# AOADMM-DataFusionFramework/Matlab-Code

Hardware: AMD Instinct MI355X
Metric: AO-ADMM outer iters/sec (+ mode-1 MTTKRP GFLOP/s), 2000^3 rank-20 CP (higher is better)
Workload: dtype f32

## Files before the change

### matlab-code_amd/csrc/contract.h

```cpp
#pragma once
#include "common.h"

namespace aoadmm {

struct DenseTensor {
  int prec = AOADMM_PREC_F64;
  int nd = 0;
  int64_t dims[8] = {0};
  int64_t pad0 = 0;
  DevBuf data;
  int64_t elems_padded() const {
    int64_t n = pad0;
    for (int i = 1; i < nd; ++i) n *= dims[i];
    return n;
  }
  size_t elem_size() const { return prec == AOADMM_PREC_F32 ? 4 : 8; }
};

struct ContractPlan {
  int64_t nbatch, batch_stride, M, ld, C;
  int R;
  int tprec = AOADMM_PREC_F64;
  int nchunk;
  bool lead = false;
  bool on_copy = false;
  int64_t trows() const { return nbatch * M; }
  size_t t_bytes() const { return (size_t)nchunk * trows() * R * (tprec == AOADMM_PREC_F32 ? 4 : 8); }
  size_t frag_bytes(int prec) const;
  double algorithmic_bytes(int prec) const {
    return (double)nbatch * M * C * (prec == AOADMM_PREC_F32 ? 4.0 : 8.0) + (double)t_bytes();
  }
  double flops() const { return 2.0 * nbatch * M * C * R; }
};

ContractPlan make_plan(int64_t nbatch, int64_t batch_stride, int64_t M, int64_t ld, int64_t C, int R,
                       int prec);

ContractPlan make_lead_plan(int64_t M, int64_t ld, int64_t C, int R);

void launch_contract(const void* X, int prec, const ContractPlan& pl, const double* F, int64_t ldF,
                     void* frag_ws, void* T, hipStream_t s, hipEvent_t ev0 = nullptr,
                     hipEvent_t ev1 = nullptr);

size_t reduce_factor_scratch_bytes(int64_t rows, int R);
struct SysBuild;
bool launch_reduce_inner(const void* T, int tprec, int nchunk, int64_t trows, int64_t A, int64_t Apad,
                         int64_t B, int R, const double* Fa, int64_t ldFa, double scale,
                         double* out, int64_t ldOut, double* ft_scratch, hipStream_t s,
                         const double* FaT = nullptr,
                         int rowmajor_out = 0,
                         const SysBuild* sys = nullptr);
size_t reduce_outer_scratch_bytes(int64_t A, int64_t B, int R);
bool launch_reduce_outer(const void* T, int tprec, int nchunk, int64_t trows, int64_t A, int64_t Apad,
                         int64_t B, int R, const double* Fb, int64_t ldFb, double scale,
                         double* out, int64_t ldOut, double* scratch, double* ft_scratch, hipStream_t s,
                         const double* FbT = nullptr, int rowmajor_out = 0, const SysBuild* sys = nullptr);
void launch_t_to_colmajor(const void* T, int tprec, int nchunk, int64_t trows, int64_t A, int R, double scale,
                          double* out, int64_t ldOut, hipStream_t s);

constexpr int64_t kSmallMttkrpElems = (int64_t)1 << 19;
struct SmallMttkrp {
  const void* X;
  int64_t sn, sa, sb;
  int Na, Nb, R;
  const double *Fa, *Fb;
  int64_t lda, ldb;
  double scale;
  double* out;
  int64_t ldOut;
};
bool small_mttkrp_ok(int64_t elems, int nd, const int64_t* dims, int R);
// ... 4 lines not shown
```

### matlab-code_amd/csrc/contract.hip

```cpp
#include "contract.h"
#include "device_utils.h"
#include "small_dev.h"

#include <algorithm>
#include <cstdlib>

namespace aoadmm {

typedef float f32x4 __attribute__((ext_vector_type(4)));
typedef double f64x2 __attribute__((ext_vector_type(2)));
typedef double f64x4 __attribute__((ext_vector_type(4)));

static constexpr int kTileRows = 128;
static constexpr int kGroup = 8;

struct KArgs {
  const void* X;
  const void* frag;
  void* T;
  int64_t tiles_per_batch, ntiles, batch_stride, M, ld, C, Cg, trows;
  int groups_per_chunk, R;
  int flush_every;
};

typedef float f32x2 __attribute__((ext_vector_type(2)));

__global__ void pack_frag16_f32(const double* __restrict__ F, int64_t ldF, int64_t C, int R, int NT, int EX,
                                int64_t Cg, float* __restrict__ frag) {
  const int64_t idx = (int64_t)blockIdx.x * blockDim.x + threadIdx.x;
  const int64_t nmain = (int64_t)NT * Cg * 128;
  if (idx < nmain) {
    const int kk = idx & 1;
    const int lane = (idx >> 1) & 63;
    const int64_t g = (idx >> 7) % Cg;
    const int nt = (int)((idx >> 7) / Cg);
    const int64_t c = 8 * g + 4 * kk + (lane >> 4);
    const int r = 16 * nt + (lane & 15);
// ... 6 lines not shown
    const int r = 16 * NT + e;
    frag[idx] = (c < C && r < R) ? (float)F[c + ldF * r] : 0.f;
  }
}

__device__ __forceinline__ float quarter_sum4(float a, float b, float c, float d) {
  const auto ab = __builtin_amdgcn_permlane16_swap(__float_as_uint(a), __float_as_uint(b), false, false);
  const auto cd = __builtin_amdgcn_permlane16_swap(__float_as_uint(c), __float_as_uint(d), false, false);
  const float s_ab = __uint_as_float(ab[0]) + __uint_as_float(ab[1]);
  const float s_cd = __uint_as_float(cd[0]) + __uint_as_float(cd[1]);
  const auto x = __builtin_amdgcn_permlane32_swap(__float_as_uint(s_ab), __float_as_uint(s_cd), false, false);
  return __uint_as_float(x[0]) + __uint_as_float(x[1]);
}

constexpr int kFlushEvery = 3;
template <int NT, bool EX, bool L2 = false>
__global__ __launch_bounds__(256, NT <= 2 ? 2 : 1) void contract16_f32(KArgs a) {
  static_assert(!L2 || NT == 1, "two-level accumulation exists for one 16-column tile (R <= 20)");
  const int lane = threadIdx.x & 63;
  const int64_t wt = (int64_t)blockIdx.x * 4 + (threadIdx.x >> 6);
  if (wt >= a.ntiles) return;
  const int chunk = blockIdx.y;
  const int64_t b = wt / a.tiles_per_batch;
  const int64_t m0 = (wt - b * a.tiles_per_batch) * kTileRows;
  const int r16 = lane & 15, q = lane >> 4;
  int64_t row0 = m0 + 4 * r16, row1 = m0 + 64 + 4 * r16;
  if (row0 >= a.M) row0 = m0;
  if (row1 >= a.M) row1 = m0;
  const int64_t g0 = (int64_t)chunk * a.groups_per_chunk;
  int64_t g1 = g0 + a.groups_per_chunk;
  if (g1 > a.Cg) g1 = a.Cg;
  const int64_t gfull = (a.C / kGroup < g1) ? a.C / kGroup : g1;
  const float* X = reinterpret_cast<const float*>(a.X) + b * a.batch_stride;
// ... 189 lines not shown
#pragma unroll
      for (int h = 0; h < 2; ++h)
#pragma unroll
        for (int v = 0; v < 4; ++v)
#pragma unroll
          for (int e = 0; e < 4; ++e)
            if (e < ne) tl[(64 * h + 4 * r16 + v) * a.R + 16 * NT + e] = accE[h][v][e >> 1][e & 1];
    }
  }
  {
    const int64_t rows_here = (a.M - m0 < kTileRows) ? a.M - m0 : kTileRows;
    const int n16 = (int)(rows_here * a.R / 4);
    f32x4* dst = reinterpret_cast<f32x4*>(reinterpret_cast<float*>(a.T) + ((int64_t)chunk * a.trows + b * a.M + m0) * a.R);
    const f32x4* src = reinterpret_cast<const f32x4*>(tl);
    for (int c = lane; c < n16; c += 64) __builtin_nontemporal_store(src[c], dst + c);
  }
}

static constexpr int kLeadRows = 128;
static constexpr int kLeadKC = 64;
static constexpr int kLeadStride = 68;

struct LArgs {
  const float* X;
  const float* frag;
  float* T;
  int64_t M, ld, C, Cg;
  int chunks_per_slice;
  int R;
};
// ... 392 lines not shown
  if (nt16 == 1) AO_SET(contract_lead16_f32<1>)
  else if (nt16 == 2) AO_SET(contract_lead16_f32<2>)
  else if (nt16 == 3) AO_SET(contract_lead16_f32<3>)
  else if (nt16 == 4) AO_SET(contract_lead16_f32<4>)
#undef AO_SET
  if (ev0) AO_HIP(hipEventRecord(ev0, s));
  if (nt16 == 1) contract_lead16_f32<1><<<grid, 256, sh, s>>>(a);
  else if (nt16 == 2) contract_lead16_f32<2><<<grid, 256, sh, s>>>(a);
  else if (nt16 == 3) contract_lead16_f32<3><<<grid, 256, sh, s>>>(a);
  else if (nt16 == 4) contract_lead16_f32<4><<<grid, 256, sh, s>>>(a);
  else throw Error(AOADMM_ERR_UNSUPPORTED, "rank > 64 not supported");
  if (ev1) AO_HIP(hipEventRecord(ev1, s));
  AO_KERNEL_CHECK();
}

void launch_contract(const void* X, int prec, const ContractPlan& pl, const double* F, int64_t ldF,
                     void* frag_ws, void* T, hipStream_t s, hipEvent_t ev0, hipEvent_t ev1) {
  AO_REQUIRE(pl.tprec == prec, "contraction plan and tensor precision disagree");
  AO_REQUIRE(pl.R >= 1 && pl.R <= kMaxRank, "rank %d outside [1,%d]", pl.R, kMaxRank);
  if (pl.lead) {
    AO_REQUIRE(prec == AOADMM_PREC_F32, "leading-mode contraction exists for fp32 tensors only");
    launch_contract_lead(X, pl, F, ldF, frag_ws, T, s, ev0, ev1);
    return;
  }
  const int64_t Cg = cdiv(pl.C, kGroup);
  KArgs a;
  a.X = X; a.frag = frag_ws; a.T = T;
  a.tiles_per_batch = cdiv(pl.M, tile_rows(prec));
  a.ntiles = pl.nbatch * a.tiles_per_batch;
  a.batch_stride = pl.batch_stride; a.M = pl.M; a.ld = pl.ld; a.C = pl.C; a.Cg = Cg;
  a.trows = pl.trows();
  a.groups_per_chunk = (int)cdiv(Cg, pl.nchunk);
  a.R = pl.R;
  AO_REQUIRE(a.ntiles > 0 && pl.C > 0, "empty contraction");
  dim3 grid((unsigned)cdiv(a.ntiles, 4), (unsigned)pl.nchunk);
  AO_REQUIRE(cdiv(a.ntiles, 4) < (int64_t)2147483647, "tensor too large for one launch");
  if (prec == AOADMM_PREC_F32) {
    AO_REQUIRE(pl.ld % 4 == 0 && pl.M % 4 == 0 && pl.batch_stride % 4 == 0, "f32 layout must be padded to 4");
    const int rem = pl.R % 16;
    const bool ex = pl.R > 16 && rem >= 1 && rem <= 4;
    const int nt16 = ex ? pl.R / 16 : (pl.R + 15) / 16;
    const int64_t total = (int64_t)nt16 * Cg * 128 + (ex ? Cg * 32 : 0);
    pack_frag16_f32<<<(unsigned)cdiv(total, 256), 256, 0, s>>>(F, ldF, pl.C, pl.R, nt16, ex ? 1 : 0, Cg, (float*)frag_ws);
    AO_KERNEL_CHECK();
    size_t tsh = (size_t)4 * kTileRows * pl.R * sizeof(float);
    a.flush_every = kFlushEvery;
    if (nt16 == 1) tsh = (size_t)4 * 16384;
#define AO_GO(K) { if (tsh > 65536) ensure_dynamic_lds(reinterpret_cast<const void*>(K), (int)tsh); if (ev0) AO_HIP(hipEventRecord(ev0, s)); K<<<grid, 256, tsh, s>>>(a); }
    if (nt16 == 1 && !ex) AO_GO((contract16_f32<1, false, true>))
    else if (nt16 == 1) AO_GO((contract16_f32<1, true, true>))
    else if (nt16 == 2 && !ex) AO_GO((contract16_f32<2, false>))
    else if (nt16 == 2) AO_GO((contract16_f32<2, true>))
    else if (nt16 == 3 && !ex) AO_GO((contract16_f32<3, false>))
    else if (nt16 == 3) AO_GO((contract16_f32<3, true>))
    else if (nt16 == 4) AO_GO((contract16_f32<4, false>))
    else throw Error(AOADMM_ERR_UNSUPPORTED, "rank > 64 not supported");
#undef AO_GO
  } else {
    AO_REQUIRE(pl.ld % 2 == 0 && pl.M % 2 == 0 && pl.batch_stride % 2 == 0, "f64 layout must be padded to 2");
    const int rem = pl.R % 16;
    const bool ex = pl.R > 16 && rem >= 1 && rem <= 4;
    const int nt16 = ex ? pl.R / 16 : (pl.R + 15) / 16;
    const int64_t total = (int64_t)nt16 * Cg * 128 + (ex ? Cg * 32 : 0);
    pack_frag_f64<<<(unsigned)cdiv(total, 256), 256, 0, s>>>(F, ldF, pl.C, pl.R, nt16, ex ? 1 : 0, Cg, (double*)frag_ws);
// ... 321 lines not shown
  int SB = 1;
  const int vec = outer_vec(tprec, R);
  if (tprec == AOADMM_PREC_F32) {
    if (vec == 4) launch_outer_t<float, 4>(T, nchunk, trows, A, Apad, B, R, ft_scratch, scratch, SB, s, sys);
    else launch_outer_t<float, 1>(T, nchunk, trows, A, Apad, B, R, ft_scratch, scratch, SB, s, sys);
  } else {
    if (vec == 2) launch_outer_t<double, 2>(T, nchunk, trows, A, Apad, B, R, ft_scratch, scratch, SB, s, sys);
    else launch_outer_t<double, 1>(T, nchunk, trows, A, Apad, B, R, ft_scratch, scratch, SB, s, sys);
  }
  AO_KERNEL_CHECK();
  reduce_outer_fin<<<(unsigned)cdiv(A * R, 256), 256, 0, s>>>(scratch, SB, A, R, scale, out, ldOut, rowmajor_out);
  AO_KERNEL_CHECK();
  return sys != nullptr;
}

template <typename TT, int RMAX>
__global__ __launch_bounds__(256) void small_mttkrp_k(SmallMttkrp a, int has_sys, SysBuild sys) {
  extern __shared__ double sf[];
  if (has_sys && blockIdx.x == 0) { sys_build_rider(sys); return; }
  const int row = (int)blockIdx.x - has_sys;
  const int R = a.R, Na = a.Na, Nb = a.Nb;
  double* fa = sf;
  double* fb = sf + (size_t)Na * R;
  double* red = fb + (size_t)(Nb > 0 ? Nb : 1) * R;
  for (int e = threadIdx.x; e < Na * R; e += 256) { const int i = e / R, r = e - i * R; fa[e] = a.Fa[i + a.lda * r]; }
  for (int e = threadIdx.x; e < Nb * R; e += 256) { const int i = e / R, r = e - i * R; fb[e] = a.Fb ? a.Fb[i + a.ldb * r] : 1.0; }
  __syncthreads();
  const TT* X = reinterpret_cast<const TT*>(a.X) + (int64_t)row * a.sn;
  double acc[RMAX];
#pragma unroll
// ... 69 lines not shown
```

### matlab-code_amd/csrc/cpblock.h

```cpp
#pragma once
#include "common.h"
#include "contract.h"
#include "sparse.h"

namespace aoadmm {

struct FactorRef {
  const double* p;
  int64_t ld;
  uint64_t version;
  const double* pT = nullptr;
};

struct KernelStats {
  std::vector<std::pair<hipEvent_t, hipEvent_t>> pending;
  double ms = 0.0, bytes = 0.0, flops = 0.0;
  int64_t launches = 0, timed = 0;
};

struct LaunchTimers {
  struct Pair { hipEvent_t e0 = nullptr, e1 = nullptr; };
  std::vector<hipEvent_t> pool;
  KernelStats stats[4];
  bool profile = true;
// ... 8 lines not shown

struct BlockCtx {
  hipStream_t stream;
  LaunchTimers* timers;
  int rank, world;
  bool sharded;
  bool allow_copies;
  DevBuf* staging;
  void (*allreduce_from)(void* comm, const double* send, double* recv, int64_t n);
  void* comm;
};

struct PassCopy {
  DevBuf buf;
  int64_t pad = 0;
  bool present = false, refused = false;
};

struct CpBlock {
  DenseTensor X;
  DenseTensor Xt;
  PassCopy copy[3];
  DevBuf emkr, emkr2;
  bool xp_ksharded = false;
  int64_t xp_k0 = 0, xp_kloc = 0;
  int nd = 0;
  int64_t dims[8] = {0};
  int64_t full0 = 0;
  int64_t row0 = 0;
  bool has_data = false;
  bool x_released = false;
  int cached_mode = -1;
  uint64_t cached_version = 0;
  ContractPlan plan;
  DevBuf T, frag, scratch, ft, tmpA, tmpB;
  DevBuf own[2];
  size_t own_bytes[2] = {0, 0};
  int64_t own_row0[2] = {-1, -1};
  DevBuf mask, maskT;
  bool has_mask = false;
  bool sparse = false;
  CooBlock coo;
  void reset_derived() {
    has_data = true; x_released = false; cached_mode = -1; xp_ksharded = false;
    for (PassCopy& c : copy) c.present = c.refused = false;
  }
};

inline int64_t pad_of(int prec, int64_t n) { return round_up(n, prec == AOADMM_PREC_F32 ? 4 : 2); }
int next_update_distance(int pos, int c, const int* seq, int n);
inline bool small_direct(bool sharded, const CpBlock& b, int R) {
  return !sharded && small_mttkrp_ok(b.X.elems_padded(), b.nd, b.dims, R);
}

void block_upload(const BlockCtx& cx, CpBlock& b, int nd, const int64_t* dims, const double* host, int prec, int64_t row0,
                  int64_t local_rows, const double* full_array = nullptr);
void adopt_ksharded_xp(const BlockCtx& cx, CpBlock& b, const void* slab, int64_t k0, int64_t kloc);
bool want_ksharded_xp(const BlockCtx& cx, const CpBlock& b, int64_t K, int64_t* k0, int64_t* kloc);
bool ensure_pass_copy(const BlockCtx& cx, CpBlock& b, int c);
// ... 10 lines not shown
```

### matlab-code_amd/csrc/cpblock.hip

```cpp
#include "cpblock.h"
#include "misc.h"

#include <algorithm>
#include <cstdlib>

namespace aoadmm {

hipEvent_t LaunchTimers::take_event() {
  if (pool.empty()) {
    for (int i = 0; i < 64; ++i) {
      hipEvent_t e = nullptr;
      AO_HIP(hipEventCreate(&e));
      pool.push_back(e);
    }
  }
  hipEvent_t e = pool.back();
  pool.pop_back();
  return e;
}

void LaunchTimers::fold_finished(KernelStats& ks) {
  size_t keep = 0;
  for (size_t i = 0; i < ks.pending.size(); ++i) {
    auto& pr = ks.pending[i];
// ... 24 lines not shown
}

void LaunchTimers::end(KernelStats& ks, Pair pr, hipStream_t s, double bytes, double flops) {
  if (pr.e0) AO_HIP(hipEventRecord(pr.e1, s));
  count(ks, pr, bytes, flops);
}

void LaunchTimers::count(KernelStats& ks, Pair pr, double bytes, double flops) {
  if (pr.e0) { ks.pending.emplace_back(pr.e0, pr.e1); ks.timed++; }
  ks.launches++;
  ks.bytes += bytes;
  ks.flops += flops;
}

static void timed_contract(const BlockCtx& cx, const void* X, int prec, const ContractPlan& pl, const double* F, int64_t ldF,
                           void* frag, void* T) {
  LaunchTimers& tm = *cx.timers;
  KernelStats& ks = tm.stats[pl.lead ? 1 : 0];
  LaunchTimers::Pair pr;
  static const bool no_events = getenv("AOADMM_NO_PASS_EVENTS") != nullptr;
  static const int every = [] { const char* e = getenv("AOADMM_PASS_EVENT_EVERY"); const int v = e ? atoi(e) : 4; return v < 1 ? 1 : v; }();
  if (tm.profile && !no_events && ks.launches % every == 0) pr = tm.take_pair(ks);
  launch_contract(X, prec, pl, F, ldF, frag, T, cx.stream, pr.e0, pr.e1);
  tm.count(ks, pr, pl.algorithmic_bytes(prec), pl.flops());
}

static size_t blocked_bytes(int64_t M, int64_t C, size_t es) { return (size_t)round_up(M, kRowBlockElems) * C * es; }

static void upload_padded(const BlockCtx& cx, void* dst, int prec, int64_t pad, const double* host, int64_t rows, int64_t ncols) {
  DevBuf& staging = *cx.staging;
  const int64_t chunk_cols = std::max<int64_t>(1, (int64_t)(64ll << 20) / rows);
  staging.ensure((size_t)std::min(chunk_cols, ncols) * rows * sizeof(double));
  for (int64_t c0 = 0; c0 < ncols; c0 += chunk_cols) {
    const int64_t nc = std::min(chunk_cols, ncols - c0);
    AO_HIP(hipMemcpyAsync(staging.p, host + c0 * rows, (size_t)nc * rows * sizeof(double), hipMemcpyHostToDevice, cx.stream));
    pad_convert(dst, prec, pad, staging.d(), rows, nc, c0, cx.stream);
    AO_HIP(hipStreamSynchronize(cx.stream));
  }
}
// ... 49 lines not shown
}

bool want_ksharded_xp(const BlockCtx& cx, const CpBlock& b, int64_t K, int64_t* k0, int64_t* kloc) {
  if (!cx.sharded || cx.world <= 1 || !cx.allow_copies || b.has_mask || b.nd != 3) return false;
  const int64_t per = cdiv(K, cx.world);
  if (per * (cx.world - 1) >= K) return false;
  *k0 = per * cx.rank;
  *kloc = std::min<int64_t>(K, *k0 + per) - *k0;
  return true;
}
void adopt_ksharded_xp(const BlockCtx& cx, CpBlock& b, const void* slab, int64_t k0, int64_t kloc) {
  const int64_t Ifull = b.full0, J = b.dims[1];
  const int prec = b.X.prec;
  PassCopy& pc = b.copy[0];
  pc.pad = pad_of(prec, J);
  pc.buf.alloc(blocked_bytes(pc.pad * kloc, Ifull, b.X.elem_size()));
  AO_REQUIRE(block_layout_copy(slab, pc.buf.p, 1, prec, Ifull, pad_of(prec, Ifull), J, kloc, pc.pad, cx.stream),
             "tensor mode too long for the copy kernels");
  pc.present = true; b.xp_ksharded = true; b.xp_k0 = k0; b.xp_kloc = kloc;
}

bool ensure_pass_copy(const BlockCtx& cx, CpBlock& b, int c) {
  PassCopy& pc = b.copy[c];
  if (pc.present) return true;
  if (pc.refused) return false;
  if (c == 1 ? !ensure_pass_copy(cx, b, 0) : (!cx.allow_copies || b.has_mask || b.nd != 3)) return false;
  const int64_t I = b.dims[0], J = b.dims[1], K = b.dims[2];
  const int64_t pad = c == 0 ? pad_of(b.X.prec, J) : (c == 1 ? pad_of(b.X.prec, K) : b.X.pad0);
  const size_t bytes = blocked_bytes(pad * b.dims[(c + 2) % 3], b.dims[c], b.X.elem_size());
  if (!room_for(bytes)) { pc.refused = true; return false; }
  pc.buf.alloc(bytes);
  pc.pad = pad;
  if (!block_layout_copy(b.X.data.p, pc.buf.p, (c + 1) % 3, b.X.prec, I, b.X.pad0, J, K, c == 2 ? 0 : pad, cx.stream)) {
    pc.buf.release(); pc.refused = true; return false;
  }
  pc.present = true;
  return true;
}

void maybe_release_natural(const BlockCtx& cx, CpBlock& b, bool normsq_valid) {
  const bool all_copies = b.copy[0].present && b.copy[1].present && b.copy[2].present;
  if (b.sparse || b.x_released || b.nd != 3 || !all_copies || b.has_mask || !normsq_valid || !b.X.data.p) return;
  const char* pe = getenv("AOADMM_RELEASE_NATURAL");
  const int policy = pe ? (atoi(pe) != 0 ? 1 : -1) : 0;
  if (policy < 0) return;
  if (policy == 0) {
    size_t free_b = 0, total_b = 0;
    const size_t mine = (size_t)b.X.elems_padded() * b.X.elem_size();
    if (hipMemGetInfo(&free_b, &total_b) != hipSuccess || free_b >= mine) return;
  }
  AO_HIP(hipStreamSynchronize(cx.stream));
  b.X.data.release();
  b.x_released = true;
}

void drop_pass_copies(CpBlock& b) {
  for (int c = 0; c < 3; ++c) {
    PassCopy& pc = b.copy[c];
    if (!pc.present) continue;
    pc.buf.release(); pc.present = false; b.cached_mode = -1;
    if (c == 0) b.xp_ksharded = false;
  }
}

int next_update_distance(int pos, int c, const int* seq, int n) {
  if (!seq || n <= 0) return c;
  int at = -1;
  for (int i = 0; i < n; ++i)
    if (seq[i] == pos) at = i;
  if (at < 0) return c;
  for (int d = 1; d <= n; ++d)
    if (seq[(at + d) % n] == c) return d;
  return n + 1;
}

// ... 1 lines not shown
                        const int* update_seq, int nseq) {
  const int prec = b.X.prec;
  const int64_t I = b.dims[0], Ip = b.X.pad0, J = b.dims[1], K = b.dims[2];
  if (b.x_released) use_cache = true;
  const bool hit = use_cache && b.cached_mode >= 0 && b.cached_mode != pos &&
                   facs[b.cached_mode].version == b.cached_version;
  if (hit) return;
  int c = -1, best = -1;
  for (int cand = 2; cand >= 0; --cand) {
    if (cand == pos) continue;
    if (cand == 0 && !(use_cache && (prec == AOADMM_PREC_F32 || ensure_pass_copy(cx, b, 0)))) continue;
    const int dist = next_update_distance(pos, cand, update_seq, nseq);
    if (dist > best) { best = dist; c = cand; }
  }
  ContractPlan pl;
  const double* Fc = c == 0 ? facs[0].p + (cx.sharded ? b.row0 : 0) : facs[c].p;
  if (use_cache && ensure_pass_copy(cx, b, c)) {
    const bool ksh = c == 0 && b.xp_ksharded;
    const int64_t M = b.copy[c].pad * (ksh ? b.xp_kloc : b.dims[(c + 2) % 3]), C = ksh ? b.full0 : b.dims[c];
    const int64_t MB = kRowBlockElems;
    pl = make_plan(round_up(M, MB) / MB, MB * C, MB, MB, C, R, prec);
    pl.on_copy = true;
    if (ksh) Fc = facs[0].p;
  } else {
    if (c == 2) pl = make_plan(1, 0, Ip * J, Ip * J, K, R, prec);
    else if (c == 1) pl = make_plan(K, Ip * J, Ip, Ip, J, R, prec);
    else pl = make_lead_plan(J * K, Ip, I, R);
  }
  b.T.ensure(pl.t_bytes()); b.frag.ensure(pl.frag_bytes(prec));
  timed_contract(cx, pl.on_copy ? b.copy[c].buf.p : b.X.data.p, prec, pl, Fc, facs[c].ld, b.frag.p, b.T.p);
  b.cached_mode = c; b.cached_version = facs[c].version; b.plan = pl;
}

struct MttkrpOut { double* p; int64_t ld; const double* send; };

static MttkrpOut own_rows_buffer(const BlockCtx& cx, CpBlock& b, int which, int64_t rows_full, int64_t row_first, int R) {
  DevBuf& ob = b.own[which];
  const size_t need = (size_t)rows_full * R * sizeof(double);
  if (b.own_bytes[which] != need || b.own_row0[which] != row_first) {
    if (b.own_bytes[which] != need) ob.alloc(need);
    AO_HIP(hipMemsetAsync(ob.p, 0, need, cx.stream));
    b.own_bytes[which] = need;
    b.own_row0[which] = row_first;
  }
  return MttkrpOut{ob.d() + row_first, rows_full, ob.d()};
}
// ... 32 lines not shown
  b.T.ensure(pl.t_bytes()); b.frag.ensure(pl.frag_bytes(prec));
  timed_contract(cx, X.data.p, prec, pl, pos == 0 ? facs[1].p : F0, facs[1 - pos].ld, b.frag.p, b.T.p);
  launch_t_to_colmajor(b.T.p, pl.tprec, pl.nchunk, pl.trows(), rows, R, scale, o.p, o.ld, cx.stream);
  b.cached_mode = -1;
}

static void mttkrp_3way(const BlockCtx& cx, CpBlock& b, int pos, const FactorRef* facs, const double* F0, int R, double scale,
                        bool use_cache, const int* update_seq, int nseq, bool sharded, MttkrpOut& o, const SysBuild* sys,
                        bool* sys_done) {
  const int64_t I = b.dims[0], Ip = b.X.pad0, J = b.dims[1], K = b.dims[2];
  ensure_contraction(cx, b, pos, facs, R, use_cache, update_seq, nseq);
  const int c = b.cached_mode;
  const ContractPlan& pl = b.plan;
  const bool ksh = sharded && pl.on_copy && c == 0 && b.xp_ksharded;
  int ia = c == 0 ? 1 : 0, ib = c == 2 ? 1 : 2;
  if (pl.on_copy && c == 1) { ia = 2; ib = 0; }
  const int64_t ext[3] = {I, J, ksh ? b.xp_kloc : K};
  const int64_t An = ext[ia], Bn = ext[ib];
  const int64_t Apad = pl.on_copy ? b.copy[c].pad : (ia == 0 ? Ip : J);
  auto fac_p = [&](int m) { return m == 0 ? F0 : (m == 2 && ksh ? facs[2].p + b.xp_k0 : facs[m].p); };
  auto fac_pT = [&](int m) -> const double* {
    if (!facs[m].pT) return nullptr;
    if (m == 2 && ksh) return facs[2].pT + b.xp_k0 * R;
    return facs[m].pT + ((m == 0 && sharded) ? b.row0 * R : 0);
  };
  if (ksh && pos == 2) o = own_rows_buffer(cx, b, 1, K, b.xp_k0, R);
  LaunchTimers& tm = *cx.timers;
  const LaunchTimers::Pair pr = tm.begin(tm.stats[2], tm.profile && tm.profile_reductions, cx.stream);
  bool rode;
  if (pos == ia) {
    b.scratch.ensure(reduce_outer_scratch_bytes(An, Bn, R));
    b.ft.ensure(reduce_factor_scratch_bytes(Bn, R));
    rode = launch_reduce_outer(b.T.p, pl.tprec, pl.nchunk, pl.trows(), An, Apad, Bn, R, fac_p(ib), facs[ib].ld, scale,
                               o.p, o.ld, b.scratch.d(), b.ft.d(), cx.stream, fac_pT(ib), 0, sys);
  } else {
    AO_REQUIRE(pos == ib, "internal: cached contraction cannot serve this mode");
    b.ft.ensure(reduce_factor_scratch_bytes(An, R));
    rode = launch_reduce_inner(b.T.p, pl.tprec, pl.nchunk, pl.trows(), An, Apad, Bn, R, fac_p(ia), facs[ia].ld, scale,
                               o.p, o.ld, b.ft.d(), cx.stream, fac_pT(ia), 0, sys);
  }
  if (sys_done) *sys_done = rode;
// ... 103 lines not shown
```

### matlab-code_amd/csrc/misc.h

```cpp
#pragma once
#include "common.h"
#include "contract.h"
#include "small.h"

namespace aoadmm {

void pad_convert(void* dst, int prec, int64_t pad_rows, const double* src, int64_t rows, int64_t cols,
                 int64_t dst_col0, hipStream_t s);
void transpose_convert(void* dst, int prec, int64_t pad_c, const double* src, int64_t rows, int64_t cols,
                       hipStream_t s);
void tensor_sumsq(double* slot, const void* X, int prec, int64_t n, double* ws, hipStream_t s);

struct SynthArgs {
  int64_t I_loc, I_pad, J, K, row0, I_full;
  int R;
  uint64_t seed;
  int64_t k0 = 0, K_loc = -1;
};
void synth_factors(double* A, double* B, double* C, const SynthArgs& a, hipStream_t s);
void synth_norms(double* out3, const double* A, const double* B, const double* C, const SynthArgs& a,
                 double* ws, hipStream_t s);
void synth_write(void* X, int prec, const double* A, const double* B, const double* C, const SynthArgs& a,
                 double sigma, double inv_norm, hipStream_t s);
size_t synth_ws_bytes();

void reg_value(double* slot, int type, double p0, const double* X, int64_t rows, int R, double* ws,
               hipStream_t s);

constexpr int64_t kRowBlockElems = 512;
bool block_layout_copy(const void* X, void* D, int which, int prec, int64_t I, int64_t Ip, int64_t J, int64_t K,
                       int64_t Tp, hipStream_t s);
struct UnfoldGramArgs {
  const void* X;
  int64_t n, sa, n1, s1, n2, s2;
};
size_t unfold_gram_ws_bytes(const UnfoldGramArgs& a);
void unfold_gram(const UnfoldGramArgs& a, int prec, double* ws, double* out, hipStream_t s);

void kr_merge(double* out, const double* Fa, int64_t lda, int64_t A, const double* Fb, int64_t ldb, int64_t B, int R,
              hipStream_t s);

}
```

### matlab-code_amd/csrc/misc.hip

```cpp
#include "misc.h"

#include <map>
#include <mutex>
#include <utility>

namespace aoadmm {

void ensure_dynamic_lds(const void* kernel, int bytes) {
  static std::mutex mu;
  static std::map<std::pair<int, const void*>, int> granted;
  int dev = 0;
  AO_HIP(hipGetDevice(&dev));
  std::lock_guard<std::mutex> lk(mu);
  int& have = granted[std::make_pair(dev, kernel)];
  if (have >= bytes) return;
  AO_HIP(hipFuncSetAttribute(kernel, hipFuncAttributeMaxDynamicSharedMemorySize, bytes));
  have = bytes;
}


template <typename T>
__global__ void pad_convert_k(T* dst, int64_t pad_rows, const double* src, int64_t rows, int64_t cols,
                              int64_t dst_col0) {
  const int64_t total = pad_rows * cols;
// ... 212 lines not shown

template <typename T>
__global__ __launch_bounds__(256) void block_copy_k(const T* __restrict__ X, T* __restrict__ D, int64_t M, int64_t Mpad,
                                                   int64_t K, int64_t MB) {
  const int64_t k = blockIdx.y;
  constexpr int V = 16 / sizeof(T);
  typedef T VT __attribute__((ext_vector_type(V)));
  for (int64_t m = ((int64_t)blockIdx.x * 256 + threadIdx.x) * V; m < Mpad; m += (int64_t)gridDim.x * 256 * V) {
    VT v;
#pragma unroll
    for (int e = 0; e < V; ++e) v[e] = (T)0;
    if (m < M) v = *reinterpret_cast<const VT*>(X + M * k + m);
    *reinterpret_cast<VT*>(D + (m / MB) * MB * K + k * MB + m % MB) = v;
  }
}
template <typename T, int WHICH>
__global__ __launch_bounds__(256) void block_permute_k(const T* __restrict__ X, T* __restrict__ D, int64_t I, int64_t Ip,
                                                      int64_t J, int64_t K, int64_t Tp, int64_t MB) {
  __shared__ T tile[32][33];
  const int64_t u = blockIdx.z;
  const int64_t i0 = (int64_t)blockIdx.x * 32, t0 = (int64_t)blockIdx.y * 32;
  const int tx = threadIdx.x & 31, ty = threadIdx.x >> 5;
  const int64_t nT = WHICH == 1 ? J : K;
  const int64_t st = WHICH == 1 ? Ip : Ip * J, su = WHICH == 1 ? Ip * J : Ip;
#pragma unroll
  for (int q = 0; q < 4; ++q) {
    const int64_t i = i0 + tx, t = t0 + ty + 8 * q;
    tile[ty + 8 * q][tx] = (i < I && t < nT) ? X[i + st * t + su * u] : (T)0;
  }
  __syncthreads();
  const int64_t C = WHICH == 1 ? I : J;
#pragma unroll
  for (int q = 0; q < 4; ++q) {
    const int64_t t = t0 + tx, i = i0 + ty + 8 * q;
    if (t < Tp && i < I) {
      const int64_t m = WHICH == 1 ? t + Tp * u : t + Tp * i;
      const int64_t c = WHICH == 1 ? i : u;
      D[(m / MB) * MB * C + c * MB + m % MB] = tile[tx][ty + 8 * q];
    }
  }
}
bool block_layout_copy(const void* X, void* D, int which, int prec, int64_t I, int64_t Ip, int64_t J, int64_t K,
                       int64_t Tp, hipStream_t s) {
  const int64_t MB = kRowBlockElems;
  const size_t es = prec == AOADMM_PREC_F32 ? 4 : 8;
  if (which == 0) {
    if (K > 65535) return false;
    const int64_t M = Ip * J, Mpad = round_up(M, MB);
    const int V = (int)(16 / es);
    int64_t gx = cdiv(Mpad, (int64_t)256 * V);
    if (gx > 65535) gx = 65535;
    const dim3 grid((unsigned)gx, (unsigned)K);
    if (prec == AOADMM_PREC_F32) block_copy_k<float><<<grid, 256, 0, s>>>((const float*)X, (float*)D, M, Mpad, K, MB);
    else block_copy_k<double><<<grid, 256, 0, s>>>((const double*)X, (double*)D, M, Mpad, K, MB);
    AO_KERNEL_CHECK();
    return true;
  }
  const int64_t nU = which == 1 ? K : J, C = which == 1 ? I : J;
  const int64_t M = which == 1 ? Tp * K : Tp * I, Mpad = round_up(M, MB);
  if (nU > 65535 || cdiv(Tp, 32) > 65535) return false;
  if (Mpad > M)
    AO_HIP(hipMemsetAsync((char*)D + (size_t)(Mpad / MB - 1) * MB * C * es, 0, (size_t)MB * C * es, s));
  const dim3 grid((unsigned)cdiv(I, 32), (unsigned)cdiv(Tp, 32), (unsigned)nU);
#define AO_BP(TT, W) block_permute_k<TT, W><<<grid, 256, 0, s>>>((const TT*)X, (TT*)D, I, Ip, J, K, Tp, MB)
  if (prec == AOADMM_PREC_F32) { if (which == 1) AO_BP(float, 1); else AO_BP(float, 2); }
  else { if (which == 1) AO_BP(double, 1); else AO_BP(double, 2); }
#undef AO_BP
  AO_KERNEL_CHECK();
  return true;
}

template <typename T>
__global__ __launch_bounds__(256) void unfold_gram_k(UnfoldGramArgs a, double* ws) {
  __shared__ double As[16][65], Bs[16][65];
  const T* X = reinterpret_cast<const T*>(a.X);
  const int tid = threadIdx.x, tx = tid & 15, ty = tid >> 4;
  const int64_t a0 = (int64_t)blockIdx.x * 64, b0 = (int64_t)blockIdx.y * 64;
  const int64_t nch1 = (a.n1 + 15) / 16, nchunks = nch1 * a.n2;
  const int64_t per = (nchunks + gridDim.z - 1) / gridDim.z;
  const int64_t c_lo = (int64_t)blockIdx.z * per;
  int64_t c_hi = c_lo + per;
// ... 92 lines not shown
```

Measured before the change: 129.1.

## Fuse first MTTKRP reduction into contraction epilogue with swapped pass-copy layouts

Adds an epilogue to the two-level f32 contraction kernel that multiplies each tile of T against the row-major factor and writes per-tile partial sums, plus a small finishing kernel that sums the partials into the MTTKRP output. This replaces the separate reduce pass that would otherwise reread T for one of the two modes sharing the cached contraction. To make the fused mode line up, pass copies in the unsharded case are now built with swapped row-mode order, using new copy/permute kernel variants. The cost is extra work and LDS use in the contraction kernel, a partials buffer, and version tracking to decide when the fused result can be reused.

```diff
diff --git a/matlab-code_amd/csrc/contract.h b/matlab-code_amd/csrc/contract.h
--- a/matlab-code_amd/csrc/contract.h
+++ b/matlab-code_amd/csrc/contract.h
@@ -38,9 +38,21 @@
 
 ContractPlan make_lead_plan(int64_t M, int64_t ld, int64_t C, int R);
 
+struct FusedFirst {
+  const double* Fa;
+  int64_t ldFa;
+  const double* FaT;
+  double* ft_scratch;
+  int64_t A, Apad, B;
+  double* partial;
+};
+bool fused_first_ok(const ContractPlan& pl, int prec, int64_t Apad);
+size_t fused_partial_bytes(const ContractPlan& pl);
+
 void launch_contract(const void* X, int prec, const ContractPlan& pl, const double* F, int64_t ldF,
                      void* frag_ws, void* T, hipStream_t s, hipEvent_t ev0 = nullptr,
-                     hipEvent_t ev1 = nullptr);
+                     hipEvent_t ev1 = nullptr,
+                     const FusedFirst* fuse = nullptr);
 
 size_t reduce_factor_scratch_bytes(int64_t rows, int R);
 struct SysBuild;
@@ -55,6 +67,8 @@
                          int64_t B, int R, const double* Fb, int64_t ldFb, double scale,
                          double* out, int64_t ldOut, double* scratch, double* ft_scratch, hipStream_t s,
                          const double* FbT = nullptr, int rowmajor_out = 0, const SysBuild* sys = nullptr);
+bool launch_fused_fin(const double* partial, const ContractPlan& pl, int64_t Apad, int64_t B, double scale, double* out,
+                      int64_t ldOut, hipStream_t s, const SysBuild* sys = nullptr);
 void launch_t_to_colmajor(const void* T, int tprec, int nchunk, int64_t trows, int64_t A, int R, double scale,
                           double* out, int64_t ldOut, hipStream_t s);
 
diff --git a/matlab-code_amd/csrc/contract.hip b/matlab-code_amd/csrc/contract.hip
--- a/matlab-code_amd/csrc/contract.hip
+++ b/matlab-code_amd/csrc/contract.hip
@@ -21,6 +21,9 @@
   int64_t tiles_per_batch, ntiles, batch_stride, M, ld, C, Cg, trows;
   int groups_per_chunk, R;
   int flush_every;
+  const double* faT = nullptr;
+  double* partial = nullptr;
+  int64_t fA = 0, fApad = 0, fMtot = 0;
 };
 
 typedef float f32x2 __attribute__((ext_vector_type(2)));
@@ -57,9 +60,11 @@
 }
 
 constexpr int kFlushEvery = 3;
-template <int NT, bool EX, bool L2 = false>
+constexpr int kFuseRowsPerLane = 44;
+template <int NT, bool EX, bool L2 = false, bool FUSE = false>
 __global__ __launch_bounds__(256, NT <= 2 ? 2 : 1) void contract16_f32(KArgs a) {
   static_assert(!L2 || NT == 1, "two-level accumulation exists for one 16-column tile (R <= 20)");
+  static_assert(!FUSE || L2, "the fused first MTTKRP exists for the two-level kernels (R <= 20)");
   const int lane = threadIdx.x & 63;
   const int64_t wt = (int64_t)blockIdx.x * 4 + (threadIdx.x >> 6);
   if (wt >= a.ntiles) return;
@@ -279,6 +284,46 @@
     f32x4* dst = reinterpret_cast<f32x4*>(reinterpret_cast<float*>(a.T) + ((int64_t)chunk * a.trows + b * a.M + m0) * a.R);
     const f32x4* src = reinterpret_cast<const f32x4*>(tl);
     for (int c = lane; c < n16; c += 64) __builtin_nontemporal_store(src[c], dst + c);
+  }
+  if (FUSE) {
+    const int R = a.R, G = 64 / R;
+    const int rg = lane / R, r = lane - rg * R;
+    const int64_t mt = wt * kTileRows;
+    const int64_t bb0 = mt / a.fApad;
+    const int64_t a0 = mt - bb0 * a.fApad;
+    const int split = a.fApad - a0 < kTileRows ? (int)(a.fApad - a0) : kTileRows;
+    const int64_t live = a.fMtot - mt;
+    double s0 = 0.0, s1 = 0.0;
+#pragma unroll
+    for (int bt = 0; bt < kFuseRowsPerLane; bt += 11) {
+      double f[11];
+      float t[11];
+#pragma unroll
+      for (int u = 0; u < 11; ++u) {
+        const int row = rg + (bt + u) * G;
+        const int64_t aa = row < split ? a0 + row : row - split;
+        const bool ok = rg < G && row < kTileRows && aa < a.fA && row < live;
+        f[u] = a.faT[ok ? aa * R + r : 0];
+        t[u] = ok ? tl[row * R + r] : 0.f;
+      }
+      __builtin_amdgcn_sched_barrier(0);
+#pragma unroll
+      for (int u = 0; u < 11; ++u) {
+        const bool second = rg + (bt + u) * G >= split;
+        s0 += (double)(second ? 0.f : t[u]) * f[u];
+        s1 += (double)(second ? t[u] : 0.f) * f[u];
+      }
+    }
+    double* red = reinterpret_cast<double*>(t_lds) + (threadIdx.x >> 6) * 2048 + 1536;
+    red[lane] = s0;
+    red[64 + lane] = s1;
+    if (lane < R) {
+      double u0 = 0.0, u1 = 0.0;
+      for (int g2 = 0; g2 < G; ++g2) { u0 += red[g2 * R + lane]; u1 += red[64 + g2 * R + lane]; }
+      double* pp = a.partial + (((int64_t)chunk * a.ntiles + wt) * 2) * R + lane;
+      pp[0] = u0;
+      pp[R] = u1;
+    }
   }
 }
 
@@ -701,10 +746,21 @@
   AO_KERNEL_CHECK();
 }
 
+static void factor_rowmajor(const double* F, int64_t ldF, int64_t rows, int R, double* Ft, hipStream_t s);
+
+static int64_t fused_tiles(const ContractPlan& pl) { return pl.nbatch * cdiv(pl.M, kTileRows); }
+bool fused_first_ok(const ContractPlan& pl, int prec, int64_t Apad) {
+  return prec == AOADMM_PREC_F32 && !pl.lead && pl.R <= 20 && pl.M % kTileRows == 0 && Apad >= kTileRows;
+}
+size_t fused_partial_bytes(const ContractPlan& pl) {
+  return (size_t)pl.nchunk * fused_tiles(pl) * 2 * pl.R * sizeof(double);
+}
+
 void launch_contract(const void* X, int prec, const ContractPlan& pl, const double* F, int64_t ldF,
-                     void* frag_ws, void* T, hipStream_t s, hipEvent_t ev0, hipEvent_t ev1) {
+                     void* frag_ws, void* T, hipStream_t s, hipEvent_t ev0, hipEvent_t ev1, const FusedFirst* fuse) {
   AO_REQUIRE(pl.tprec == prec, "contraction plan and tensor precision disagree");
   AO_REQUIRE(pl.R >= 1 && pl.R <= kMaxRank, "rank %d outside [1,%d]", pl.R, kMaxRank);
+  AO_REQUIRE(!fuse || fused_first_ok(pl, prec, fuse->Apad), "internal: this pass cannot sum the first MTTKRP");
   if (pl.lead) {
     AO_REQUIRE(prec == AOADMM_PREC_F32, "leading-mode contraction exists for fp32 tensors only");
     launch_contract_lead(X, pl, F, ldF, frag_ws, T, s, ev0, ev1);
@@ -733,8 +789,17 @@
     size_t tsh = (size_t)4 * kTileRows * pl.R * sizeof(float);
     a.flush_every = kFlushEvery;
     if (nt16 == 1) tsh = (size_t)4 * 16384;
+    if (fuse) {
+      AO_REQUIRE(fuse->Apad * fuse->B <= pl.trows() && fuse->A <= fuse->Apad, "internal: fused MTTKRP rows outside the pass");
+      if (!fuse->FaT) factor_rowmajor(fuse->Fa, fuse->ldFa, fuse->A, pl.R, fuse->ft_scratch, s);
+      a.faT = fuse->FaT ? fuse->FaT : fuse->ft_scratch;
+      a.partial = fuse->partial;
+      a.fA = fuse->A; a.fApad = fuse->Apad; a.fMtot = fuse->Apad * fuse->B;
+    }
 #define AO_GO(K) { if (tsh > 65536) ensure_dynamic_lds(reinterpret_cast<const void*>(K), (int)tsh); if (ev0) AO_HIP(hipEventRecord(ev0, s)); K<<<grid, 256, tsh, s>>>(a); }
-    if (nt16 == 1 && !ex) AO_GO((contract16_f32<1, false, true>))
+    if (nt16 == 1 && !ex && fuse) AO_GO((contract16_f32<1, false, true, true>))
+    else if (nt16 == 1 && fuse) AO_GO((contract16_f32<1, true, true, true>))
+    else if (nt16 == 1 && !ex) AO_GO((contract16_f32<1, false, true>))
     else if (nt16 == 1) AO_GO((contract16_f32<1, true, true>))
     else if (nt16 == 2 && !ex) AO_GO((contract16_f32<2, false>))
     else if (nt16 == 2) AO_GO((contract16_f32<2, true>))
@@ -1086,6 +1151,42 @@
   return sys != nullptr;
 }
 
+__global__ __launch_bounds__(256) void fused_first_fin_k(const double* __restrict__ part, int nchunk, int64_t ntiles,
+                                                        int64_t Apad, int64_t B, int R, double scale,
+                                                        double* __restrict__ out, int64_t ldOut, int has_sys, SysBuild sys) {
+  if (has_sys && blockIdx.x == 0) { sys_build_rider(sys); return; }
+  const int64_t idx = ((int64_t)blockIdx.x - has_sys) * 256 + threadIdx.x;
+  if (idx >= B * R) return;
+  const int64_t bb = idx / R;
+  const int r = (int)(idx - bb * R);
+  const int64_t m0 = Apad * bb, t0 = m0 / kTileRows, t1 = (m0 + Apad - 1) / kTileRows;
+  double tot = 0.0;
+  for (int ch = 0; ch < nchunk; ++ch) {
+    const double* pc = part + (int64_t)ch * ntiles * 2 * R + r;
+    int64_t t = t0;
+    for (; t + 7 <= t1; t += 8) {
+      double v[8];
+#pragma unroll
+      for (int u = 0; u < 8; ++u) v[u] = pc[((t + u) * 2 + ((t + u) * kTileRows < m0 ? 1 : 0)) * R];
+#pragma unroll
+      for (int u = 0; u < 8; ++u) tot += v[u];
+    }
+    for (; t <= t1; ++t) tot += pc[(t * 2 + (t * kTileRows < m0 ? 1 : 0)) * R];
+  }
+  out[bb + ldOut * r] = scale * tot;
+}
+
+bool launch_fused_fin(const double* partial, const ContractPlan& pl, int64_t Apad, int64_t B, double scale, double* out,
+                      int64_t ldOut, hipStream_t s, const SysBuild* sys) {
+  if (!sys_can_ride(sys, 256)) sys = nullptr;
+  const int hs = sys ? 1 : 0;
+  AO_REQUIRE(B * pl.R < (int64_t)2147483647 * 256, "fused MTTKRP: too many output rows for one launch");
+  fused_first_fin_k<<<(unsigned)(cdiv(B * pl.R, 256) + hs), 256, 0, s>>>(partial, pl.nchunk, fused_tiles(pl), Apad, B, pl.R,
+                                                                         scale, out, ldOut, hs, sys ? *sys : SysBuild());
+  AO_KERNEL_CHECK();
+  return sys != nullptr;
+}
+
 template <typename TT, int RMAX>
 __global__ __launch_bounds__(256) void small_mttkrp_k(SmallMttkrp a, int has_sys, SysBuild sys) {
   extern __shared__ double sf[];
diff --git a/matlab-code_amd/csrc/cpblock.h b/matlab-code_amd/csrc/cpblock.h
--- a/matlab-code_amd/csrc/cpblock.h
+++ b/matlab-code_amd/csrc/cpblock.h
@@ -46,6 +46,7 @@
 struct PassCopy {
   DevBuf buf;
   int64_t pad = 0;
+  int ma = -1, mb = -1;
   bool present = false, refused = false;
 };
 
@@ -66,6 +67,9 @@
   uint64_t cached_version = 0;
   ContractPlan plan;
   DevBuf T, frag, scratch, ft, tmpA, tmpB;
+  int fused_pos = -1;
+  uint64_t fused_version = 0;
+  DevBuf partial;
   DevBuf own[2];
   size_t own_bytes[2] = {0, 0};
   int64_t own_row0[2] = {-1, -1};
@@ -74,7 +78,7 @@
   bool sparse = false;
   CooBlock coo;
   void reset_derived() {
-    has_data = true; x_released = false; cached_mode = -1; xp_ksharded = false;
+    has_data = true; x_released = false; cached_mode = -1; fused_pos = -1; xp_ksharded = false;
     for (PassCopy& c : copy) c.present = c.refused = false;
   }
 };
diff --git a/matlab-code_amd/csrc/cpblock.hip b/matlab-code_amd/csrc/cpblock.hip
--- a/matlab-code_amd/csrc/cpblock.hip
+++ b/matlab-code_amd/csrc/cpblock.hip
@@ -62,15 +62,15 @@
 }
 
 static void timed_contract(const BlockCtx& cx, const void* X, int prec, const ContractPlan& pl, const double* F, int64_t ldF,
-                           void* frag, void* T) {
+                           void* frag, void* T, const FusedFirst* fuse = nullptr) {
   LaunchTimers& tm = *cx.timers;
   KernelStats& ks = tm.stats[pl.lead ? 1 : 0];
   LaunchTimers::Pair pr;
   static const bool no_events = getenv("AOADMM_NO_PASS_EVENTS") != nullptr;
   static const int every = [] { const char* e = getenv("AOADMM_PASS_EVENT_EVERY"); const int v = e ? atoi(e) : 4; return v < 1 ? 1 : v; }();
   if (tm.profile && !no_events && ks.launches % every == 0) pr = tm.take_pair(ks);
-  launch_contract(X, prec, pl, F, ldF, frag, T, cx.stream, pr.e0, pr.e1);
-  tm.count(ks, pr, pl.algorithmic_bytes(prec), pl.flops());
+  launch_contract(X, prec, pl, F, ldF, frag, T, cx.stream, pr.e0, pr.e1, fuse);
+  tm.count(ks, pr, pl.algorithmic_bytes(prec) + (fuse ? (double)fused_partial_bytes(pl) : 0.0), pl.flops());
 }
 
 static size_t blocked_bytes(int64_t M, int64_t C, size_t es) { return (size_t)round_up(M, kRowBlockElems) * C * es; }
@@ -150,6 +150,7 @@
   const int prec = b.X.prec;
   PassCopy& pc = b.copy[0];
   pc.pad = pad_of(prec, J);
+  pc.ma = 1; pc.mb = 2;
   pc.buf.alloc(blocked_bytes(pc.pad * kloc, Ifull, b.X.elem_size()));
   AO_REQUIRE(block_layout_copy(slab, pc.buf.p, 1, prec, Ifull, pad_of(prec, Ifull), J, kloc, pc.pad, cx.stream),
              "tensor mode too long for the copy kernels");
@@ -162,12 +163,14 @@
   if (pc.refused) return false;
   if (c == 1 ? !ensure_pass_copy(cx, b, 0) : (!cx.allow_copies || b.has_mask || b.nd != 3)) return false;
   const int64_t I = b.dims[0], J = b.dims[1], K = b.dims[2];
-  const int64_t pad = c == 0 ? pad_of(b.X.prec, J) : (c == 1 ? pad_of(b.X.prec, K) : b.X.pad0);
-  const size_t bytes = blocked_bytes(pad * b.dims[(c + 2) % 3], b.dims[c], b.X.elem_size());
+  const bool swap = !cx.sharded;
+  const int ma = swap ? (c + 2) % 3 : (c + 1) % 3, mb = swap ? (c + 1) % 3 : (c + 2) % 3;
+  const int64_t pad = ma == 0 ? b.X.pad0 : pad_of(b.X.prec, b.dims[ma]);
+  const size_t bytes = blocked_bytes(pad * b.dims[mb], b.dims[c], b.X.elem_size());
   if (!room_for(bytes)) { pc.refused = true; return false; }
   pc.buf.alloc(bytes);
-  pc.pad = pad;
-  if (!block_layout_copy(b.X.data.p, pc.buf.p, (c + 1) % 3, b.X.prec, I, b.X.pad0, J, K, c == 2 ? 0 : pad, cx.stream)) {
+  pc.pad = pad; pc.ma = ma; pc.mb = mb;
+  if (!block_layout_copy(b.X.data.p, pc.buf.p, (c + 1) % 3, b.X.prec, I, b.X.pad0, J, K, pad, cx.stream, swap)) {
     pc.buf.release(); pc.refused = true; return false;
   }
   pc.present = true;
@@ -194,7 +197,7 @@
   for (int c = 0; c < 3; ++c) {
     PassCopy& pc = b.copy[c];
     if (!pc.present) continue;
-    pc.buf.release(); pc.present = false; b.cached_mode = -1;
+    pc.buf.release(); pc.present = false; b.cached_mode = -1; b.fused_pos = -1;
     if (c == 0) b.xp_ksharded = false;
   }
 }
@@ -226,22 +229,35 @@
     if (dist > best) { best = dist; c = cand; }
   }
   ContractPlan pl;
+  FusedFirst fuse;
+  bool fused = false;
   const double* Fc = c == 0 ? facs[0].p + (cx.sharded ? b.row0 : 0) : facs[c].p;
   if (use_cache && ensure_pass_copy(cx, b, c)) {
     const bool ksh = c == 0 && b.xp_ksharded;
-    const int64_t M = b.copy[c].pad * (ksh ? b.xp_kloc : b.dims[(c + 2) % 3]), C = ksh ? b.full0 : b.dims[c];
+    const PassCopy& pc = b.copy[c];
+    const int64_t M = pc.pad * (ksh ? b.xp_kloc : b.dims[pc.mb]), C = ksh ? b.full0 : b.dims[c];
     const int64_t MB = kRowBlockElems;
     pl = make_plan(round_up(M, MB) / MB, MB * C, MB, MB, C, R, prec);
     pl.on_copy = true;
     if (ksh) Fc = facs[0].p;
+    if (!cx.sharded && pos == pc.mb && fused_first_ok(pl, prec, pc.pad)) {
+      const FactorRef& fa = facs[pc.ma];
+      if (!fa.pT) b.ft.ensure(reduce_factor_scratch_bytes(b.dims[pc.ma], R));
+      b.partial.ensure(fused_partial_bytes(pl));
+      fuse = FusedFirst{fa.p, fa.ld, fa.pT, b.ft.d(), b.dims[pc.ma], pc.pad, b.dims[pc.mb], b.partial.d()};
+      fused = true;
+      b.fused_version = fa.version;
+    }
   } else {
     if (c == 2) pl = make_plan(1, 0, Ip * J, Ip * J, K, R, prec);
     else if (c == 1) pl = make_plan(K, Ip * J, Ip, Ip, J, R, prec);
     else pl = make_lead_plan(J * K, Ip, I, R);
   }
   b.T.ensure(pl.t_bytes()); b.frag.ensure(pl.frag_bytes(prec));
-  timed_contract(cx, pl.on_copy ? b.copy[c].buf.p : b.X.data.p, prec, pl, Fc, facs[c].ld, b.frag.p, b.T.p);
+  timed_contract(cx, pl.on_copy ? b.copy[c].buf.p : b.X.data.p, prec, pl, Fc, facs[c].ld, b.frag.p, b.T.p,
+                 fused ? &fuse : nullptr);
   b.cached_mode = c; b.cached_version = facs[c].version; b.plan = pl;
+  b.fused_pos = fused ? pos : -1;
 }
 
 struct MttkrpOut { double* p; int64_t ld; const double* send; };
@@ -304,7 +320,7 @@
   const ContractPlan& pl = b.plan;
   const bool ksh = sharded && pl.on_copy && c == 0 && b.xp_ksharded;
   int ia = c == 0 ? 1 : 0, ib = c == 2 ? 1 : 2;
-  if (pl.on_copy && c == 1) { ia = 2; ib = 0; }
+  if (pl.on_copy) { ia = b.copy[c].ma; ib = b.copy[c].mb; }
   const int64_t ext[3] = {I, J, ksh ? b.xp_kloc : K};
   const int64_t An = ext[ia], Bn = ext[ib];
   const int64_t Apad = pl.on_copy ? b.copy[c].pad : (ia == 0 ? Ip : J);
@@ -315,6 +331,11 @@
     return facs[m].pT + ((m == 0 && sharded) ? b.row0 * R : 0);
   };
   if (ksh && pos == 2) o = own_rows_buffer(cx, b, 1, K, b.xp_k0, R);
+  if (pl.on_copy && b.fused_pos == pos && pos == ib && facs[ia].version == b.fused_version) {
+    const bool rode = launch_fused_fin(b.partial.d(), pl, Apad, Bn, scale, o.p, o.ld, cx.stream, sys);
+    if (sys_done) *sys_done = rode;
+    return;
+  }
   LaunchTimers& tm = *cx.timers;
   const LaunchTimers::Pair pr = tm.begin(tm.stats[2], tm.profile && tm.profile_reductions, cx.stream);
   bool rode;
diff --git a/matlab-code_amd/csrc/misc.h b/matlab-code_amd/csrc/misc.h
--- a/matlab-code_amd/csrc/misc.h
+++ b/matlab-code_amd/csrc/misc.h
@@ -29,7 +29,7 @@
 
 constexpr int64_t kRowBlockElems = 512;
 bool block_layout_copy(const void* X, void* D, int which, int prec, int64_t I, int64_t Ip, int64_t J, int64_t K,
-                       int64_t Tp, hipStream_t s);
+                       int64_t Tp, hipStream_t s, bool swap_rows = false);
 struct UnfoldGramArgs {
   const void* X;
   int64_t n, sa, n1, s1, n2, s2;
diff --git a/matlab-code_amd/csrc/misc.hip b/matlab-code_amd/csrc/misc.hip
--- a/matlab-code_amd/csrc/misc.hip
+++ b/matlab-code_amd/csrc/misc.hip
@@ -250,37 +250,51 @@
     *reinterpret_cast<VT*>(D + (m / MB) * MB * K + k * MB + m % MB) = v;
   }
 }
+template <typename T>
+__global__ __launch_bounds__(256) void block_swap_copy_k(const T* __restrict__ X, T* __restrict__ D, int64_t Ip, int64_t J,
+                                                        int64_t MB) {
+  const int64_t j = blockIdx.y, k = blockIdx.z;
+  constexpr int V = 16 / sizeof(T);
+  typedef T VT __attribute__((ext_vector_type(V)));
+  const T* src = X + Ip * (j + J * k);
+  for (int64_t i = ((int64_t)blockIdx.x * 256 + threadIdx.x) * V; i < Ip; i += (int64_t)gridDim.x * 256 * V) {
+    const int64_t m = i + Ip * k;
+    *reinterpret_cast<VT*>(D + (m / MB) * MB * J + j * MB + m % MB) = *reinterpret_cast<const VT*>(src + i);
+  }
+}
 template <typename T, int WHICH>
 __global__ __launch_bounds__(256) void block_permute_k(const T* __restrict__ X, T* __restrict__ D, int64_t I, int64_t Ip,
                                                       int64_t J, int64_t K, int64_t Tp, int64_t MB) {
   __shared__ T tile[32][33];
+  constexpr bool TJ = WHICH == 1 || WHICH == 3;
+  constexpr bool CI = WHICH == 1 || WHICH == 4;
   const int64_t u = blockIdx.z;
   const int64_t i0 = (int64_t)blockIdx.x * 32, t0 = (int64_t)blockIdx.y * 32;
   const int tx = threadIdx.x & 31, ty = threadIdx.x >> 5;
-  const int64_t nT = WHICH == 1 ? J : K;
-  const int64_t st = WHICH == 1 ? Ip : Ip * J, su = WHICH == 1 ? Ip * J : Ip;
+  const int64_t nT = TJ ? J : K;
+  const int64_t st = TJ ? Ip : Ip * J, su = TJ ? Ip * J : Ip;
 #pragma unroll
   for (int q = 0; q < 4; ++q) {
     const int64_t i = i0 + tx, t = t0 + ty + 8 * q;
     tile[ty + 8 * q][tx] = (i < I && t < nT) ? X[i + st * t + su * u] : (T)0;
   }
   __syncthreads();
-  const int64_t C = WHICH == 1 ? I : J;
+  const int64_t C = CI ? I : (TJ ? K : J);
 #pragma unroll
   for (int q = 0; q < 4; ++q) {
     const int64_t t = t0 + tx, i = i0 + ty + 8 * q;
     if (t < Tp && i < I) {
-      const int64_t m = WHICH == 1 ? t + Tp * u : t + Tp * i;
-      const int64_t c = WHICH == 1 ? i : u;
+      const int64_t m = CI ? t + Tp * u : t + Tp * i;
+      const int64_t c = CI ? i : u;
       D[(m / MB) * MB * C + c * MB + m % MB] = tile[tx][ty + 8 * q];
     }
   }
 }
 bool block_layout_copy(const void* X, void* D, int which, int prec, int64_t I, int64_t Ip, int64_t J, int64_t K,
-                       int64_t Tp, hipStream_t s) {
+                       int64_t Tp, hipStream_t s, bool swap_rows) {
   const int64_t MB = kRowBlockElems;
   const size_t es = prec == AOADMM_PREC_F32 ? 4 : 8;
-  if (which == 0) {
+  if (which == 0 && !swap_rows) {
     if (K > 65535) return false;
     const int64_t M = Ip * J, Mpad = round_up(M, MB);
     const int V = (int)(16 / es);
@@ -292,15 +306,34 @@
     AO_KERNEL_CHECK();
     return true;
   }
-  const int64_t nU = which == 1 ? K : J, C = which == 1 ? I : J;
-  const int64_t M = which == 1 ? Tp * K : Tp * I, Mpad = round_up(M, MB);
+  if (which == 2 && swap_rows) {
+    if (J > 65535 || K > 65535) return false;
+    const int64_t M = Ip * K, Mpad = round_up(M, MB);
+    if (Mpad > M)
+      AO_HIP(hipMemsetAsync((char*)D + (size_t)(Mpad / MB - 1) * MB * J * es, 0, (size_t)MB * J * es, s));
+    const int V = (int)(16 / es);
+    int64_t gx = cdiv(Ip, (int64_t)256 * V);
+    if (gx > 65535) gx = 65535;
+    const dim3 grid((unsigned)gx, (unsigned)J, (unsigned)K);
+    if (prec == AOADMM_PREC_F32) block_swap_copy_k<float><<<grid, 256, 0, s>>>((const float*)X, (float*)D, Ip, J, MB);
+    else block_swap_copy_k<double><<<grid, 256, 0, s>>>((const double*)X, (double*)D, Ip, J, MB);
+    AO_KERNEL_CHECK();
+    return true;
+  }
+  const int form = !swap_rows ? which : (which == 0 ? 3 : 4);
+  const bool tj = form == 1 || form == 3, ci = form == 1 || form == 4;
+  const int64_t nU = tj ? K : J, C = ci ? I : nU;
+  const int64_t M = ci ? Tp * nU : Tp * I, Mpad = round_up(M, MB);
   if (nU > 65535 || cdiv(Tp, 32) > 65535) return false;
   if (Mpad > M)
     AO_HIP(hipMemsetAsync((char*)D + (size_t)(Mpad / MB - 1) * MB * C * es, 0, (size_t)MB * C * es, s));
   const dim3 grid((unsigned)cdiv(I, 32), (unsigned)cdiv(Tp, 32), (unsigned)nU);
 #define AO_BP(TT, W) block_permute_k<TT, W><<<grid, 256, 0, s>>>((const TT*)X, (TT*)D, I, Ip, J, K, Tp, MB)
-  if (prec == AOADMM_PREC_F32) { if (which == 1) AO_BP(float, 1); else AO_BP(float, 2); }
-  else { if (which == 1) AO_BP(double, 1); else AO_BP(double, 2); }
+  if (prec == AOADMM_PREC_F32) {
+    if (form == 1) AO_BP(float, 1); else if (form == 2) AO_BP(float, 2); else if (form == 3) AO_BP(float, 3); else AO_BP(float, 4);
+  } else {
+    if (form == 1) AO_BP(double, 1); else if (form == 2) AO_BP(double, 2); else if (form == 3) AO_BP(double, 3); else AO_BP(double, 4);
+  }
 #undef AO_BP
   AO_KERNEL_CHECK();
   return true;
```

After: 129.1 (median of 2 runs). Within noise of the previous version (-0.0%).
